# ChainSafe/Spectre

Measured on NVIDIA H100. Metric: bn254_g1_msm_pairs_per_s, higher is better.
Workload: dtype u256 (8x32-bit Montgomery limbs, INT32 IMAD)

## Files before the change

### spectre_b200/csrc/capi.cu

```cuda
#include "common.cuh"
#include "ntt.cuh"
#include "../../include/spectre_b200.h"
#include <stdarg.h>
#include <stdio.h>
#include <sys/types.h>
#include <stdlib.h>
#include <string.h>

using namespace spb;

static_assert(sizeof(spb_fr) == sizeof(Fr) && sizeof(spb_g1_affine) == sizeof(G1Affine) && sizeof(spb_g1) == sizeof(G1Jac),
              "C ABI structs must match the device structs byte for byte");

namespace spb {

int set_error(spb_ctx* ctx, int code, const char* fmt, ...) {
  char buf[512];
  va_list ap; va_start(ap, fmt); vsnprintf(buf, sizeof buf, fmt, ap); va_end(ap);
  if (ctx) ctx->last_error = buf;
  return code;
}

void* slot(spb_ctx* ctx, DeviceState& d, const char* name, size_t bytes) {
  DevBuf& b = d.slots[name];
// ... 78 lines not shown

}

template <class P>
__global__ void field_op_kernel(int op, const Fp<P>* a, const Fp<P>* b, Fp<P>* o, size_t n) {
  size_t i = blockIdx.x * (size_t)blockDim.x + threadIdx.x;
  if (i >= n) return;
  Fp<P> x = a[i], y = b[i], r;
  if (op == 0) r = fp_mul(x, y);
  else if (op == 1) r = fp_add(x, y);
  else r = fp_sub(x, y);
  o[i] = r;
}

template <class P, int ILP, bool SQR = false>
__global__ void modmul_bench_kernel(Fp<P>* out, uint32_t iters) {
  Fp<P> x[ILP], y;
  uint32_t tid = blockIdx.x * blockDim.x + threadIdx.x;
#pragma unroll
  for (int j = 0; j < ILP; j++) { x[j] = fp_one<P>(); x[j].l[0] ^= tid * 2654435761u + j; x[j].l[7] &= 0x0fffffffu; }
  y = x[0]; y.l[1] ^= 0x9e3779b9u;
  for (uint32_t i = 0; i < iters; i++) {
#pragma unroll
    for (int j = 0; j < ILP; j++) x[j] = SQR ? fp_sqr(x[j]) : fp_mul(x[j], y);
  }
  Fp<P> acc = x[0];
#pragma unroll
  for (int j = 1; j < ILP; j++) acc = fp_add(acc, x[j]);
  out[tid] = acc;
}

extern "C" {

int spb_device_count(void) {
  int n = 0;
  if (cudaGetDeviceCount(&n) != cudaSuccess) return 0;
  return n;
}

spb_ctx* spb_init(const int* device_ids, int n_dev) {
  int avail = spb_device_count();
  if (n_dev <= 0) n_dev = 1;
  if (avail <= 0) { fprintf(stderr, "spectre_b200: no CUDA device visible; this library has no CPU fallback\n"); return nullptr; }
  spb_ctx* ctx = new spb_ctx();
  for (int i = 0; i < n_dev; i++) {
    int id = device_ids ? device_ids[i] : i;
    if (id < 0 || id >= avail) { fprintf(stderr, "spectre_b200: device id %d out of range (have %d)\n", id, avail); delete ctx; return nullptr; }
    DeviceState d; d.device = id;
    if (cudaSetDevice(id) != cudaSuccess) { delete ctx; return nullptr; }
    cudaDeviceProp prop;
    if (cudaGetDeviceProperties(&prop, id) != cudaSuccess) { delete ctx; return nullptr; }
    d.sm_count = prop.multiProcessorCount;
    d.total_mem = prop.totalGlobalMem;
    if (cudaStreamCreateWithFlags(&d.stream, cudaStreamNonBlocking) != cudaSuccess) { delete ctx; return nullptr; }
    cudaEventCreate(&d.ev0); cudaEventCreate(&d.ev1);
    cudaEventCreateWithFlags(&d.dep_ev, cudaEventDisableTiming);
    for (int e = 0; e < 8; e++) cudaEventCreate(&d.stage_ev[e]);
    d.pinned_cap = 1 << 20;
    if (cudaMallocHost(&d.pinned, d.pinned_cap) != cudaSuccess) { delete ctx; return nullptr; }
    ctx->dev.push_back(d);
  }
  ctx->peer_access = ctx->dev.size() > 1;
  for (size_t i = 0; i < ctx->dev.size(); i++)
    for (size_t j = 0; j < ctx->dev.size(); j++) {
      if (i == j) continue;
      int can = 0;
      cudaDeviceCanAccessPeer(&can, ctx->dev[i].device, ctx->dev[j].device);
      if (!can) { ctx->peer_access = false; continue; }
      cudaSetDevice(ctx->dev[i].device);
      cudaError_t e = cudaDeviceEnablePeerAccess(ctx->dev[j].device, 0);
      if (e != cudaSuccess && e != cudaErrorPeerAccessAlreadyEnabled) ctx->peer_access = false;
      cudaGetLastError();
    }
  if (!ctx->dev.empty()) cudaSetDevice(ctx->dev[0].device);
  return ctx;
}

void spb_shutdown(spb_ctx* ctx) {
  if (!ctx) return;
  msm_release_ctx(ctx);
  for (auto& d : ctx->dev) {
    cudaSetDevice(d.device);
    cudaStreamSynchronize(d.stream);
    for (auto& kv : d.slots) if (kv.second.ptr) cudaFree(kv.second.ptr);
    ntt_free_tables(d);
    if (d.pinned) cudaFreeHost(d.pinned);
    for (int i = 0; i < 2; i++) { if (d.stage[i]) cudaFreeHost(d.stage[i]); if (d.stage_done[i]) cudaEventDestroy(d.stage_done[i]); }
    cudaEventDestroy(d.ev0); cudaEventDestroy(d.ev1); cudaEventDestroy(d.dep_ev);
    for (int e = 0; e < 8; e++) cudaEventDestroy(d.stage_ev[e]);
    cudaStreamDestroy(d.stream);
  }
  delete ctx;
}

int spb_release_workspace(spb_ctx* ctx) {
  if (!ctx) return SPB_ERR_ARG;
  std::lock_guard<std::mutex> lk(ctx->mu);
  if (ctx->shplonk_slots_busy) return set_error(ctx, SPB_ERR_STATE, "spb_release_workspace: an spb_shplonk handle is open");
  for (auto& d : ctx->dev) {
    SPB_CUDA(ctx, cudaSetDevice(d.device));
    SPB_CUDA(ctx, cudaDeviceSynchronize());
    for (auto& kv : d.slots) if (kv.second.ptr) cudaFree(kv.second.ptr);
    d.slots.clear();
    ntt_free_tables(d);
  }
  if (!ctx->dev.empty()) cudaSetDevice(ctx->dev[0].device);
// ... 301 lines not shown
```

### spectre_b200/csrc/common.cuh

```cuda
#pragma once
#include <cuda_runtime.h>
#include <stdint.h>
#include <stdio.h>
#include <string.h>
#include <initializer_list>
#include <map>
#include <mutex>
#include <string>
#include <vector>
#include "curve.cuh"
#include "../../include/spectre_b200.h"

namespace spb {


struct DevBuf {
  void* ptr = nullptr;
  size_t cap = 0;
};

struct NttTables {
  Fr omega;
  uint32_t k, h;
  Fr* tw_lo = nullptr;
  Fr* tw_hi = nullptr;
  Fr* tw_full = nullptr;
};

struct MsmLane {
  cudaStream_t stream = nullptr;
  cudaEvent_t ev[9] = {nullptr, nullptr, nullptr, nullptr, nullptr, nullptr, nullptr, nullptr, nullptr};
  void* pinned = nullptr;
  bool ready = false;
};
static const int kMaxMsmLanes = 3;

struct DeviceState {
  int device = 0;
  int sm_count = 0;
  size_t total_mem = 0;
  cudaStream_t stream = nullptr;
  cudaEvent_t ev0 = nullptr, ev1 = nullptr;
  cudaEvent_t dep_ev = nullptr;
  cudaEvent_t stage_ev[8] = {nullptr, nullptr, nullptr, nullptr, nullptr, nullptr, nullptr, nullptr};
  std::map<std::string, DevBuf> slots;
  MsmLane lanes[kMaxMsmLanes];
  std::vector<NttTables> ntt_tables;
  std::vector<NttTables> ntt_pre_tables;
  void* pinned = nullptr;
  size_t pinned_cap = 0;
  void* stage[2] = {nullptr, nullptr};
  cudaEvent_t stage_done[2] = {nullptr, nullptr};
};

}

struct spb_ctx {
  std::vector<spb::DeviceState> dev;
  std::mutex mu;
  std::string last_error;
  bool peer_access = false;
  uint64_t n_kernel_launches = 0;
  float last_kernel_ms = 0.f;
  uint64_t last_msm_adds = 0;
  bool shplonk_slots_busy = false;
  float msm_stage_ms[7] = {0, 0, 0, 0, 0, 0, 0};
};

struct spb_domain {
  uint32_t j, k, extended_k, quotient_poly_degree;
  spb::Fr omega, omega_inv, extended_omega, extended_omega_inv, g_coset, g_coset_inv, ifft_divisor, extended_ifft_divisor;
  uint32_t t_len;
  spb::Fr* d_t_evaluations;
  int device;
};

namespace spb {

int set_error(spb_ctx* ctx, int code, const char* fmt, ...);
void* slot(spb_ctx* ctx, DeviceState& d, const char* name, size_t bytes);

#define SPB_CUDA(ctx, call)                                                                      \
  do {                                                                                           \
    cudaError_t e_ = (call);                                                                     \
    if (e_ != cudaSuccess) return spb::set_error(ctx, SPB_ERR_CUDA, "%s:%d %s: %s", __FILE__, __LINE__, #call, cudaGetErrorString(e_)); \
  } while (0)
#define SPB_TRY(expr)            \
  do {                           \
    int rc_ = (expr);            \
    if (rc_ != 0) return rc_;    \
  } while (0)

// ... 2 lines not shown
  DeviceState& d = (ctx)->dev[0];               \
  SPB_CUDA(ctx, cudaSetDevice(d.device));

inline unsigned nblk(uint64_t n, unsigned t) { return (unsigned)((n + t - 1) / t); }

template <class... P, class... A>
int launch(spb_ctx* ctx, cudaStream_t stream, dim3 grid, dim3 block, size_t smem, void (*kernel)(P...), const A&... args) {
  if (!grid.x || !grid.y || !grid.z) return 0;
  kernel<<<grid, block, smem, stream>>>(args...);
  ctx->n_kernel_launches++;
  const cudaError_t e = cudaGetLastError();
  if (e != cudaSuccess)
    return set_error(ctx, SPB_ERR_CUDA, "kernel launch (grid %ux%ux%u, block %u, %zu B shared memory): %s", grid.x, grid.y, grid.z,
                     block.x * block.y * block.z, smem, cudaGetErrorString(e));
  return 0;
}

struct Staging {
  const char* slot;
  size_t bytes;
  const void* in;
  void* out;
  size_t in_bytes = bytes, out_bytes = bytes;
};
template <class Core>
int run_staged(spb_ctx* ctx, DeviceState& d, std::initializer_list<Staging> bufs, Core&& core) {
  std::vector<void*> p;
  for (const Staging& b : bufs) {
    p.push_back(slot(ctx, d, b.slot, b.bytes));
    if (!p.back()) return SPB_ERR_OOM;
  }
  size_t i = 0;
  for (const Staging& b : bufs) {
    if (b.in) SPB_CUDA(ctx, cudaMemcpyAsync(p[i], b.in, b.in_bytes, cudaMemcpyHostToDevice, d.stream));
    i++;
  }
  SPB_TRY(core(p.data()));
  i = 0;
  for (const Staging& b : bufs) {
    if (b.out) SPB_CUDA(ctx, cudaMemcpyAsync(b.out, p[i], b.out_bytes, cudaMemcpyDeviceToHost, d.stream));
    i++;
  }
  SPB_CUDA(ctx, cudaStreamSynchronize(d.stream));
  return 0;
}

struct RowRange { int dev_index; uint64_t lo, hi; };
std::vector<RowRange> row_ranges(spb_ctx* ctx, uint64_t rows);

int stream_file_to_device(spb_ctx* ctx, DeviceState& d, FILE* f, void* d_dst, size_t bytes, const char* what);
int stream_device_to_file(spb_ctx* ctx, DeviceState& d, FILE* f, const void* d_src, size_t bytes, const char* what);

void msm_release_ctx(spb_ctx* ctx);

struct NttOpts {
  uint64_t n_in = 0, n_out = 0;
  const Fr* pre3 = nullptr;
  const Fr* post3 = nullptr;
  const Fr* pre_generator = nullptr;
};
void ntt_free_tables(DeviceState& d);
int ntt_device(spb_ctx* ctx, DeviceState& d, const Fr* d_src, Fr* d_dst, uint32_t log_n, const Fr& omega, const NttOpts& opts);
bool ntt_multi_applicable(spb_ctx* ctx, uint32_t log_n);
int ntt_multi_host(spb_ctx* ctx, const Fr* in, Fr* out, uint32_t log_n, const Fr& omega, const NttOpts& opts, float* ev_ms);

int dev_grand_product(spb_ctx* ctx, DeviceState& d, const Fr* da, size_t n, Fr* dz, const Fr& init);
int dev_kate_division(spb_ctx* ctx, DeviceState& d, const Fr* da, size_t n, const Fr& b, Fr* dq);
int dev_batch_invert(spb_ctx* ctx, DeviceState& d, Fr* da, size_t n);
int dev_product_enqueue(spb_ctx* ctx, DeviceState& d, const Fr* da, size_t n, Fr** d_total);
int dev_eval_polynomial(spb_ctx* ctx, DeviceState& d, const Fr* dp, size_t n, const Fr& x, Fr* out_host);

inline Fr fr_from_u64(uint64_t v) {
  Fr a = fp_zero<FrParams>(); a.l[0] = (uint32_t)v; a.l[1] = (uint32_t)(v >> 32);
  return fp_to_mont(a);
}
inline Fr fr_load(const spb_fr* p) { Fr a; memcpy(&a, p, 32); return a; }
inline Fr fr_const(const uint32_t (&v)[8]) { Fr a; for (int i = 0; i < 8; i++) a.l[i] = v[i]; return a; }
inline Fr fr_root_of_unity(uint32_t k) {
  constexpr uint32_t v[8] = SPB_FR_ROOT_OF_UNITY_MONT;
  Fr w = fr_const(v);
  for (uint32_t i = k; i < SPB_FR_S; i++) w = fp_sqr(w);
  return w;
}
inline Fr fr_zeta() { constexpr uint32_t v[8] = SPB_FR_ZETA_MONT; return fr_const(v); }
inline Fr fr_delta() { constexpr uint32_t v[8] = SPB_FR_DELTA_MONT; return fr_const(v); }

}
```

### spectre_b200/csrc/msm.cu

```cuda
#define SPB_MSM_KERNELS 1
#include "common.cuh"
#include "msm.cuh"
#include <cub/device/device_scan.cuh>
#include <string.h>

using namespace spb;

struct SrsShard {
  int dev_index = 0;
  size_t start = 0, count = 0;
  G1Affine* g = nullptr;
  G1Affine* g_lagrange = nullptr;
};
struct spb_srs {
  uint32_t k = 0;
  size_t n = 0;
  unsigned char g2[128] = {0}, s_g2[128] = {0};
  uint32_t table_c = 0;
  std::vector<SrsShard> shards;
};


namespace spb {

typedef MsmLane Lane;
static const size_t kLanePinnedBytes = 256 * 1024;
static int get_lane(spb_ctx* ctx, int dev_index, int lane_index, Lane** out) {
  Lane& l = ctx->dev[dev_index].lanes[lane_index];
  if (!l.ready) {
    SPB_CUDA(ctx, cudaStreamCreateWithFlags(&l.stream, cudaStreamNonBlocking));
    for (int i = 0; i < 9; i++) SPB_CUDA(ctx, cudaEventCreate(&l.ev[i]));
    SPB_CUDA(ctx, cudaMallocHost(&l.pinned, kLanePinnedBytes));
    l.ready = true;
  }
  *out = &l;
  return 0;
}

void msm_release_ctx(spb_ctx* ctx) {
  for (auto& d : ctx->dev) {
    cudaSetDevice(d.device);
    for (auto& l : d.lanes) {
      if (!l.ready) continue;
      cudaStreamSynchronize(l.stream);
      for (int i = 0; i < 9; i++) cudaEventDestroy(l.ev[i]);
      cudaFreeHost(l.pinned);
      cudaStreamDestroy(l.stream);
      l = Lane();
    }
  }
}

static void* lane_slot(spb_ctx* ctx, DeviceState& d, int lane, const char* name, size_t bytes) {
  char buf[64];
  snprintf(buf, sizeof buf, "%s#%d", name, lane);
  return slot(ctx, d, buf, bytes);
}

static uint32_t choose_chunk(const DeviceState& d, uint64_t est_entries) {
  const double wave = (double)d.sm_count * 512.0;
  if (est_entries >= kLongChunkMinEntries) return kLongChunk;
  double waves = (double)est_entries / 32.0 / wave;
  if (waves < 1.0) return 32;
  double w = waves < 1.5 ? 1.0 : (double)(uint64_t)(waves + 0.5);
  uint32_t L = (uint32_t)((double)est_entries / (w * wave)) + 1;
  if (L < 24) L = 24;
  if (L > 48) L = 48;
  return L;
}

static int msm_enqueue(spb_ctx* ctx, DeviceState& d, int lane, Lane& ln, const Fr* d_scalars, const G1Affine* d_bases, uint64_t n, MsmGeom g) {
  const uint64_t nb = (uint64_t)g.BW * g.B;
  const uint64_t cap = n * g.W;
  const uint32_t Lmin = g.L == kLongChunk ? kShortChunk : g.L;
  const uint64_t Tmax = (cap + Lmin - 1) / Lmin;
  if (cap >= 0x7fffffffull) return set_error(ctx, SPB_ERR_ARG, "msm: %llu entries exceed the 31-bit sort index", (unsigned long long)cap);
  uint32_t* counts = (uint32_t*)lane_slot(ctx, d, lane, "msm_counts", (nb + 1) * 4);
  uint32_t* offsets = (uint32_t*)lane_slot(ctx, d, lane, "msm_offsets", (nb + 1) * 4);
  MsmEntry* ent = (MsmEntry*)lane_slot(ctx, d, lane, "msm_entries", (cap + 1) * sizeof(MsmEntry));
  G1Xyzz* buckets = (G1Xyzz*)lane_slot(ctx, d, lane, "msm_buckets", nb * sizeof(G1Xyzz));
  uint32_t* head_key = (uint32_t*)lane_slot(ctx, d, lane, "msm_head_key", (Tmax + 1) * 4);
  uint32_t* tail_key = (uint32_t*)lane_slot(ctx, d, lane, "msm_tail_key", (Tmax + 1) * 4);
  G1Xyzz* head = (G1Xyzz*)lane_slot(ctx, d, lane, "msm_head", (Tmax + 1) * sizeof(G1Xyzz));
  G1Xyzz* tail = (G1Xyzz*)lane_slot(ctx, d, lane, "msm_tail", (Tmax + 1) * sizeof(G1Xyzz));
  uint32_t* giant = (uint32_t*)lane_slot(ctx, d, lane, "msm_giant", (Tmax + 2) * 4);
  const uint64_t max_huge = Tmax / kHugeChain + 1;
  uint32_t* huge = (uint32_t*)lane_slot(ctx, d, lane, "msm_huge", (2 * max_huge + 2) * 4);
  G1Xyzz* huge_part = (G1Xyzz*)lane_slot(ctx, d, lane, "msm_huge_part", max_huge * kHugeBlocks * sizeof(G1Xyzz));
  const MsmTail tl = msm_tail_shape(g.c);
  const uint32_t R = 1u << tl.r_log, C = 1u << tl.c_log, per = msm_tail_partials(tl);
  const uint32_t T1 = g.B >> tl.m_log;
  const uint64_t ngroups = (uint64_t)g.BW * T1;
  G1Xyzz* grp = (G1Xyzz*)lane_slot(ctx, d, lane, "msm_groups", 2 * ngroups * sizeof(G1Xyzz));
  G1Xyzz* seg_out = (G1Xyzz*)lane_slot(ctx, d, lane, "msm_rowcol", (uint64_t)g.BW * (2 * R + C) * sizeof(G1Xyzz));
  G1Xyzz* win_out = (G1Xyzz*)lane_slot(ctx, d, lane, "msm_partials", (uint64_t)g.BW * per * sizeof(G1Xyzz));
  size_t scan_bytes = 0;
  cub::DeviceScan::ExclusiveSum(nullptr, scan_bytes, counts, offsets, (int)(nb + 1), ln.stream);
  void* scan_tmp = lane_slot(ctx, d, lane, "msm_scan_tmp", scan_bytes ? scan_bytes : 16);
  if (!counts || !offsets || !ent || !buckets || !head_key || !tail_key || !head || !tail || !giant || !huge || !huge_part || !grp || !seg_out || !win_out || !scan_tmp)
    return SPB_ERR_OOM;
  if ((size_t)g.BW * per * sizeof(G1Xyzz) + 16 > kLanePinnedBytes) return set_error(ctx, SPB_ERR_STATE, "msm: %u window partials exceed the pinned staging area", g.BW * per);

  cudaStream_t st = ln.stream;
  SPB_CUDA(ctx, cudaMemsetAsync(giant, 0, 4, st));
  SPB_CUDA(ctx, cudaMemsetAsync(huge, 0, 4, st));
  const unsigned tb = 256;
  SPB_CUDA(ctx, cudaMemsetAsync(counts, 0, (nb + 1) * 4, st));
  cudaEventRecord(ln.ev[0], st);
  SPB_TRY(launch(ctx, st, nblk(n, tb), tb, 0, msm_count_kernel, n, d_scalars, g, counts));
  cudaEventRecord(ln.ev[1], st);
  SPB_CUDA(ctx, cub::DeviceScan::ExclusiveSum(scan_tmp, scan_bytes, counts, offsets, (int)(nb + 1), st));
  SPB_CUDA(ctx, cudaMemcpyAsync(counts, offsets, (nb + 1) * 4, cudaMemcpyDeviceToDevice, st));
  cudaEventRecord(ln.ev[2], st);
  SPB_TRY(launch(ctx, st, nblk(n, tb), tb, 0, msm_scatter_kernel, n, d_scalars, g, counts, ent));
  const uint32_t* total = offsets + nb;
  cudaEventRecord(ln.ev[3], st);
  SPB_TRY(launch(ctx, st, nblk(Tmax, 128), 128, 0, msm_accumulate_kernel, total, g, ent, d_bases, buckets, head_key, head, tail_key, tail));
  cudaEventRecord(ln.ev[4], st);
  SPB_TRY(launch(ctx, st, nblk(Tmax, 128), 128, 0, msm_stitch_kernel, total, g.L, 24, head_key, head, tail_key, tail, buckets, giant, giant + 1));
  SPB_TRY(launch(ctx, st, 256, 128, 0, msm_giant_kernel, total, g.L, giant, giant + 1, head_key, head, tail_key, tail, buckets, huge, huge + 2));
  SPB_TRY(launch(ctx, st, kHugeBlocks, 128, 0, msm_huge_kernel, huge, huge + 2, head, huge_part));
  SPB_TRY(launch(ctx, st, 64, 128, 0, msm_huge_finish_kernel, huge, huge + 2, kHugeBlocks, huge_part, tail_key, tail, buckets));
  cudaEventRecord(ln.ev[5], st);
  G1Xyzz *rows = seg_out, *cols = seg_out + (uint64_t)g.BW * R, *wrows = seg_out + (uint64_t)g.BW * (R + C);
  SPB_TRY(launch(ctx, st, nblk(ngroups, 128), 128, 0, msm_group_kernel, ngroups, tl.m_log, offsets, buckets, grp, grp + ngroups));
  cudaEventRecord(ln.ev[6], st);
  SPB_TRY(launch(ctx, st, g.BW * (2 * R + C), 64, 0, msm_rowcol_kernel, T1, tl, grp, grp + ngroups, rows, cols, wrows));
  SPB_TRY(launch(ctx, st, g.BW * (2 * tl.nbr + tl.nbc), 128, 0, msm_weighted_kernel, tl, rows, cols, wrows, win_out));
  cudaEventRecord(ln.ev[7], st);
  SPB_CUDA(ctx, cudaMemcpyAsync(ln.pinned, win_out, (size_t)g.BW * per * sizeof(G1Xyzz), cudaMemcpyDeviceToHost, st));
  SPB_CUDA(ctx, cudaMemcpyAsync((char*)ln.pinned + (size_t)g.BW * per * sizeof(G1Xyzz), total, 4, cudaMemcpyDeviceToHost, st));
  return 0;
}

static G1Xyzz msm_finish(Lane& ln, MsmGeom g, uint64_t* adds) {
  const MsmTail tl = msm_tail_shape(g.c);
  const uint32_t per = msm_tail_partials(tl);
  const G1Xyzz* P = (const G1Xyzz*)ln.pinned;
  uint32_t M; memcpy(&M, (const char*)ln.pinned + (size_t)g.BW * per * sizeof(G1Xyzz), 4);
  if (adds) *adds += (uint64_t)M + 2ull * g.BW * g.B;
  std::vector<G1Xyzz> S(g.BW);
  for (uint32_t w = 0; w < g.BW; w++) S[w] = msm_tail_finish(g, P + (size_t)w * per);
  return msm_combine_windows(S.data(), g.BW, g.c);
}

static void write_result(const G1Xyzz& r, spb_g1* out) {
  G1Affine a = xyzz_to_affine(r);
  G1Jac j = jac_from_affine(a);
  memcpy(out, &j, sizeof(G1Jac));
}

struct MsmPart {
  int dev_index;
  const Fr* d_scalars;
  const Fr* h_scalars;
  int peer_src_device;
  const G1Affine* d_bases;
  uint64_t n;
  MsmGeom g;
};

static int job_enqueue(spb_ctx* ctx, int lane, std::vector<MsmPart>& parts) {
  for (auto& p : parts) {
    if (!p.n) continue;
    DeviceState& d = ctx->dev[p.dev_index];
    SPB_CUDA(ctx, cudaSetDevice(d.device));
    Lane* ln; SPB_TRY(get_lane(ctx, p.dev_index, lane, &ln));
    p.g.L = choose_chunk(d, p.n * p.g.W);
    const Fr* ds = p.d_scalars;
    DeviceState& src = p.peer_src_device >= 0 ? ctx->dev[0] : d;
    if (&src != &d) SPB_CUDA(ctx, cudaSetDevice(src.device));
    SPB_CUDA(ctx, cudaEventRecord(src.dep_ev, src.stream));
    if (&src != &d) SPB_CUDA(ctx, cudaSetDevice(d.device));
// ... 363 lines not shown
    if (!src) return set_error(ctx, SPB_ERR_STATE, "spb_srs_download: basis %d not resident", basis);
    DeviceState& d = ctx->dev[sh.dev_index];
    SPB_CUDA(ctx, cudaSetDevice(d.device));
    SPB_CUDA(ctx, cudaMemcpy((G1Affine*)out + (lo - start), src + (lo - sh.start), (hi - lo) * sizeof(G1Affine), cudaMemcpyDeviceToHost));
  }
  return 0;
}

int spb_msm_raw(spb_ctx* ctx, const spb_fr* scalars, const spb_g1_affine* bases, size_t n, spb_g1* out) {
  if (!ctx || !out || (n && (!scalars || !bases))) return SPB_ERR_ARG;
  std::lock_guard<std::mutex> lk(ctx->mu);
  ctx->last_msm_adds = 0;
  std::vector<MsmPart> parts;
  size_t D = ctx->dev.size();
  for (size_t i = 0; i < D; i++) {
    size_t lo = n * i / D, cnt = n * (i + 1) / D - lo;
    if (!cnt) continue;
    DeviceState& d = ctx->dev[i];
    SPB_CUDA(ctx, cudaSetDevice(d.device));
    Lane* ln; SPB_TRY(get_lane(ctx, (int)i, 0, &ln));
    G1Affine* db = (G1Affine*)slot(ctx, d, "msm_raw_bases", cnt * sizeof(G1Affine));
    if (!db) return SPB_ERR_OOM;
    SPB_CUDA(ctx, cudaMemcpyAsync(db, (const G1Affine*)bases + lo, cnt * sizeof(G1Affine), cudaMemcpyHostToDevice, ln->stream));
    MsmPart p; p.dev_index = (int)i; p.d_scalars = nullptr; p.h_scalars = (const Fr*)scalars + lo; p.peer_src_device = -1;
    p.d_bases = db; p.n = cnt; p.g = msm_choose_geometry(cnt);
    parts.push_back(p);
  }
  SPB_TRY(job_enqueue(ctx, 0, parts));
  return job_collect(ctx, 0, parts, out);
}

static int srs_parts(spb_ctx* ctx, const spb_srs* srs, int basis, const Fr* scalars, bool on_device, size_t n, std::vector<MsmPart>& parts) {
  if (n > srs->n) return set_error(ctx, SPB_ERR_ARG, "spb_msm: %zu scalars but the SRS has %zu points", n, srs->n);
  for (auto& sh : srs->shards) {
    if (sh.start >= n) continue;
    size_t cnt = (n - sh.start) < sh.count ? (n - sh.start) : sh.count;
    const G1Affine* b = basis == SPB_BASIS_G ? sh.g : sh.g_lagrange;
    if (!b) return set_error(ctx, SPB_ERR_STATE, "spb_msm: basis %d not resident", basis);
    MsmPart p; p.dev_index = sh.dev_index; p.d_bases = b; p.n = cnt; p.h_scalars = nullptr; p.d_scalars = nullptr; p.peer_src_device = -1;
    if (!on_device) p.h_scalars = scalars + sh.start;
    else { p.d_scalars = scalars + sh.start; if (sh.dev_index != 0) p.peer_src_device = ctx->dev[0].device; }
    p.g = srs->table_c ? msm_make_geometry(srs->table_c, true, (uint32_t)sh.count) : msm_choose_geometry(cnt);
    parts.push_back(p);
  }
  return 0;
}

static int msm_batch_common(spb_ctx* ctx, const spb_srs* srs, int basis, const spb_fr* const* scalars, bool on_device, size_t n, size_t count, spb_g1* out) {
  if (!ctx || !srs || !out || (count && !scalars)) return SPB_ERR_ARG;
  std::lock_guard<std::mutex> lk(ctx->mu);
  ctx->last_msm_adds = 0;
  const MsmGeom lg = srs->table_c ? msm_make_geometry(srs->table_c, true, 0) : msm_choose_geometry(n ? n : 1);
  const uint64_t ents = (uint64_t)n * lg.W;
  const uint64_t lane_bytes = ents * sizeof(MsmEntry) + 2 * (ents / kShortChunk + 1) * (sizeof(G1Xyzz) + 4) + (uint64_t)lg.BW * lg.B * sizeof(G1Xyzz);
  const uint64_t fit = ctx->dev[0].total_mem / 10 / (lane_bytes ? lane_bytes : 1);
  const size_t NL = std::max<size_t>(1, std::min<size_t>((size_t)kMaxMsmLanes, (size_t)fit));
  std::vector<MsmPart> jobs[kMaxMsmLanes];
  for (size_t i = 0; i < count; i++) {
    int lane = (int)(i % NL);
    if (i >= NL) SPB_TRY(job_collect(ctx, lane, jobs[lane], &out[i - NL]));
    if (n && !scalars[i]) return SPB_ERR_ARG;
    jobs[lane].clear();
    SPB_TRY(srs_parts(ctx, srs, basis, (const Fr*)scalars[i], on_device, n, jobs[lane]));
    SPB_TRY(job_enqueue(ctx, lane, jobs[lane]));
  }
  for (size_t i = count >= NL ? count - NL : 0; i < count; i++) SPB_TRY(job_collect(ctx, (int)(i % NL), jobs[i % NL], &out[i]));
  return 0;
}

int spb_msm(spb_ctx* ctx, const spb_srs* srs, int basis, const spb_fr* scalars, size_t n, spb_g1* out) {
  const spb_fr* one[1] = {scalars};
  if (n && !scalars) return SPB_ERR_ARG;
  return msm_batch_common(ctx, srs, basis, one, false, n, 1, out);
}
int spb_msm_dev(spb_ctx* ctx, const spb_srs* srs, int basis, const spb_fr* d_scalars, size_t n, spb_g1* out) {
  const spb_fr* one[1] = {d_scalars};
  if (n && !d_scalars) return SPB_ERR_ARG;
  return msm_batch_common(ctx, srs, basis, one, true, n, 1, out);
}
int spb_msm_batch(spb_ctx* ctx, const spb_srs* srs, int basis, const spb_fr* const* scalars, size_t n, size_t count, spb_g1* out) {
  return msm_batch_common(ctx, srs, basis, scalars, false, n, count, out);
}
int spb_msm_batch_dev(spb_ctx* ctx, const spb_srs* srs, int basis, const spb_fr* const* d_scalars, size_t n, size_t count, spb_g1* out) {
  return msm_batch_common(ctx, srs, basis, d_scalars, true, n, count, out);
}

int spb_srs_precompute(spb_ctx* ctx, spb_srs* srs) {
  if (!ctx || !srs) return SPB_ERR_ARG;
  std::lock_guard<std::mutex> lk(ctx->mu);
  if (srs->table_c) return 0;
  size_t per_dev = srs->shards.empty() ? srs->n : srs->shards[0].count;
  uint32_t c = msm_choose_c(per_dev ? per_dev : 1, true);
  uint32_t W = (255 + c - 1) / c;
  for (auto& sh : srs->shards) {
    if (!sh.count) continue;
    SPB_CUDA(ctx, cudaSetDevice(ctx->dev[sh.dev_index].device));
    size_t free_b = 0, total_b = 0;
    SPB_CUDA(ctx, cudaMemGetInfo(&free_b, &total_b));
    const size_t bases = (sh.g ? 1 : 0) + (sh.g_lagrange ? 1 : 0);
    if ((size_t)W * sh.count * sizeof(G1Affine) * bases > total_b / 4) return 0;
  }
  for (auto& sh : srs->shards) {
    if (!sh.count) continue;
    DeviceState& d = ctx->dev[sh.dev_index];
    SPB_CUDA(ctx, cudaSetDevice(d.device));
    if ((uint64_t)W * sh.count >= 0x7fffffffull) return set_error(ctx, SPB_ERR_ARG, "spb_srs_precompute: table index exceeds 31 bits");
    for (int which = 0; which < 2; which++) {
// ... 26 lines not shown
```

### spectre_b200/csrc/msm.cuh

```cuda
#pragma once
#include <stdlib.h>
#include "curve.cuh"

namespace spb {

struct MsmGeom {
  uint32_t c;
  uint32_t W;
  uint32_t B;
  uint32_t L;
  uint32_t BW;
  uint32_t precomp;
  uint32_t tab_stride;
};

struct alignas(8) MsmEntry { uint32_t key, val; };

static const uint32_t kLongChunk = 96, kShortChunk = 32;
#ifndef SPB_LONG_CHUNK_MIN_ENTRIES
#define SPB_LONG_CHUNK_MIN_ENTRIES (1ull << 23)
#endif
static const uint64_t kLongChunkMinEntries = SPB_LONG_CHUNK_MIN_ENTRIES;
SPB_HD uint32_t msm_effective_chunk(uint32_t L, uint64_t M) { return (L == kLongChunk && M < kLongChunkMinEntries) ? kShortChunk : L; }

static const uint32_t kNoKey = 0xffffffffu;

#if defined(__CUDA_ARCH__)
SPB_D uint32_t spb_atomic_inc(uint32_t* p) { return atomicAdd(p, 1u); }
#else
inline uint32_t spb_atomic_inc(uint32_t* p) { uint32_t v = *p; *p = v + 1; return v; }
#endif

struct DigitIter {
  uint32_t limbs[8];
  uint32_t c, carry, w;
  SPB_HD void init(const Fr& canonical, uint32_t c_) {
    for (int i = 0; i < 8; i++) limbs[i] = canonical.l[i];
    c = c_; carry = 0; w = 0;
  }
  SPB_HD int32_t next() {
    uint32_t bit = w * c, word = bit >> 5, sh = bit & 31;
    uint64_t v = 0;
    if (word < 8) {
      v = limbs[word];
      if (word + 1 < 8) v |= (uint64_t)limbs[word + 1] << 32;
      v >>= sh;
    }
    uint32_t raw = (uint32_t)(v & ((1u << c) - 1)) + carry;
    w++;
    if (raw > (1u << (c - 1))) { carry = 1; return (int32_t)raw - (int32_t)(1u << c); }
    carry = 0;
    return (int32_t)raw;
  }
};

SPB_HD void msm_count_thread(uint64_t tid, uint64_t n, const Fr* scalars, MsmGeom g, uint32_t* counts) {
  if (tid >= n) return;
  Fr s = fp_from_mont(scalars[tid]);
  if (fp_is_zero(s)) return;
  DigitIter it; it.init(s, g.c);
  for (uint32_t w = 0; w < g.W; w++) {
    int32_t d = it.next();
    if (d == 0) continue;
    uint32_t mag = d < 0 ? (uint32_t)(-d) : (uint32_t)d;
    spb_atomic_inc(&counts[(g.precomp ? 0u : w * g.B) + mag - 1]);
  }
}

SPB_HD void msm_scatter_thread(uint64_t tid, uint64_t n, const Fr* scalars, MsmGeom g, uint32_t* cursor, MsmEntry* ent) {
  if (tid >= n) return;
  Fr s = fp_from_mont(scalars[tid]);
  if (fp_is_zero(s)) return;
  DigitIter it; it.init(s, g.c);
  for (uint32_t w = 0; w < g.W; w++) {
    int32_t d = it.next();
    if (d == 0) continue;
    uint32_t mag = d < 0 ? (uint32_t)(-d) : (uint32_t)d;
    uint32_t key = (g.precomp ? 0u : w * g.B) + mag - 1;
    uint32_t pos = spb_atomic_inc(&cursor[key]);
    MsmEntry e; e.key = key; e.val = ((uint32_t)tid + (g.precomp ? w * g.tab_stride : 0u)) | (d < 0 ? 0x80000000u : 0u);
    ent[pos] = e;
  }
}

SPB_HD G1Affine msm_load_point(const G1Affine* bases, uint32_t val) {
#if defined(__CUDA_ARCH__)
  const uint4* q = reinterpret_cast<const uint4*>(bases + (val & 0x7fffffffu));
  uint4 a = __ldg(q), b = __ldg(q + 1), c = __ldg(q + 2), d = __ldg(q + 3);
  G1Affine p;
  p.x.l[0] = a.x; p.x.l[1] = a.y; p.x.l[2] = a.z; p.x.l[3] = a.w; p.x.l[4] = b.x; p.x.l[5] = b.y; p.x.l[6] = b.z; p.x.l[7] = b.w;
  p.y.l[0] = c.x; p.y.l[1] = c.y; p.y.l[2] = c.z; p.y.l[3] = c.w; p.y.l[4] = d.x; p.y.l[5] = d.y; p.y.l[6] = d.z; p.y.l[7] = d.w;
#else
  G1Affine p = bases[val & 0x7fffffffu];
#endif
  if (val & 0x80000000u) p.y = fp_neg(p.y);
  return p;
}

SPB_HD MsmEntry msm_load_entry(const MsmEntry* p) {
#if defined(__CUDA_ARCH__)
  uint2 v = __ldg(reinterpret_cast<const uint2*>(p));
  MsmEntry e; e.key = v.x; e.val = v.y; return e;
#else
  return *p;
#endif
}

SPB_HD void msm_accumulate_thread(uint64_t tid, uint64_t M, MsmGeom g, const MsmEntry* ent,
                                  const G1Affine* bases, G1Xyzz* buckets, uint32_t* head_key, G1Xyzz* head,
                                  uint32_t* tail_key, G1Xyzz* tail) {
  const uint32_t L = msm_effective_chunk(g.L, M);
  uint64_t lo = tid * L;
  if (lo >= M) return;
  uint64_t hi = lo + L < M ? lo + L : M;
  uint32_t hk = kNoKey, tk = kNoKey;
  MsmEntry first = msm_load_entry(ent + lo);
  uint32_t cur = first.key;
  bool run_started_before = lo > 0 && msm_load_entry(ent + lo - 1).key == cur;
  G1Xyzz acc = xyzz_from_affine(msm_load_point(bases, first.val));
  for (uint64_t e = lo + 1; e < hi; e++) {
    MsmEntry en = msm_load_entry(ent + e);
    uint32_t k = en.key;
    G1Affine p = msm_load_point(bases, en.val);
    if (k == cur) {
      xyzz_add_mixed(acc, p);
    } else {
      if (run_started_before) { hk = cur; head[tid] = acc; }
      else buckets[cur] = acc;
      run_started_before = false;
      cur = k;
      acc = xyzz_from_affine(p);
    }
  }
  bool continues = hi < M && msm_load_entry(ent + hi).key == cur;
  if (continues) {
    if (run_started_before) { hk = cur; head[tid] = acc; }
    else { tk = cur; tail[tid] = acc; }
  } else {
    if (run_started_before) { hk = cur; head[tid] = acc; }
    else buckets[cur] = acc;
  }
  head_key[tid] = hk;
  tail_key[tid] = tk;
}

SPB_HD void msm_stitch_thread(uint64_t tid, uint64_t T, uint32_t cap, const uint32_t* head_key, const G1Xyzz* head,
                              const uint32_t* tail_key, const G1Xyzz* tail, G1Xyzz* buckets, uint32_t* giant_count,
                              uint32_t* giant_list) {
  if (tid >= T) return;
  uint32_t key = tail_key[tid];
  if (key == kNoKey) return;
  uint64_t j = tid + 1, len = 0;
  while (j < T && head_key[j] == key && len <= cap) { j++; len++; }
  if (len > cap) { uint32_t slot = spb_atomic_inc(giant_count); giant_list[slot] = (uint32_t)tid; return; }
  G1Xyzz acc = tail[tid];
  for (uint64_t q = tid + 1; q < tid + 1 + len; q++) xyzz_add(acc, head[q]);
  buckets[key] = acc;
}

struct MsmTail {
  uint32_t m_log;
  uint32_t r_log, c_log;
  uint32_t nbr, nbc;
};
inline MsmTail msm_tail_shape(uint32_t c) {
  MsmTail t; uint32_t bits = c - 1;
  t.m_log = bits < 3 ? bits : 3;
  bits -= t.m_log;
  t.c_log = bits / 2; t.r_log = bits - t.c_log;
  t.nbr = ((1u << t.r_log) + 127) / 128; t.nbc = ((1u << t.c_log) + 127) / 128;
  return t;
}
SPB_HD uint32_t msm_tail_partials(const MsmTail& t) { return 3 * t.nbr + 2 * t.nbc; }

SPB_HD void msm_group_thread(uint64_t tid, uint64_t ngroups, uint32_t m_log, const uint32_t* offsets, const G1Xyzz* buckets, G1Xyzz* s1, G1Xyzz* w1) {
  if (tid >= ngroups) return;
  const uint64_t b0 = tid << m_log;
  G1Xyzz run = xyzz_identity(), acc = xyzz_identity();
  uint32_t hi = offsets[b0 + (1u << m_log)];
  for (int j = (int)(1u << m_log) - 1; j >= 0; j--) {
    const uint32_t lo = offsets[b0 + (uint64_t)j];
    if (hi != lo) xyzz_add(run, buckets[b0 + (uint64_t)j]);
    hi = lo;
    if (j >= 1) xyzz_add(acc, run);
  }
  s1[tid] = run;
  w1[tid] = acc;
}
inline void msm_tail_host(const MsmGeom& g, const uint32_t* offsets, const G1Xyzz* buckets, G1Xyzz* partials) {
  MsmTail t = msm_tail_shape(g.c);
  uint32_t R = 1u << t.r_log, C = 1u << t.c_log, per = msm_tail_partials(t);
  const uint64_t T = (uint64_t)g.B >> t.m_log;
  G1Xyzz* s1 = (G1Xyzz*)malloc(sizeof(G1Xyzz) * T * g.BW);
  G1Xyzz* w1 = (G1Xyzz*)malloc(sizeof(G1Xyzz) * T * g.BW);
  for (uint64_t tid = 0; tid < T * g.BW; tid++) msm_group_thread(tid, T * g.BW, t.m_log, offsets, buckets, s1, w1);
  for (uint32_t w = 0; w < g.BW; w++) {
// ... 43 lines not shown
  return A;
}

#if defined(__CUDACC__) && defined(SPB_MSM_KERNELS)
__device__ __forceinline__ unsigned msm_warp_peers(uint32_t key, uint32_t lane) {
  const uint32_t next = __shfl_down_sync(0xffffffffu, key, 1);
  const bool dup = lane < 31u && next == key && key != kNoKey;
  if (__any_sync(0xffffffffu, dup)) return __match_any_sync(0xffffffffu, key);
  return 1u << lane;
}
__global__ void msm_count_kernel(uint64_t n, const Fr* scalars, MsmGeom g, uint32_t* counts) {
  const uint64_t tid = blockIdx.x * (uint64_t)blockDim.x + threadIdx.x;
  const uint32_t lane = threadIdx.x & 31u;
  bool live = tid < n;
  Fr s = live ? fp_from_mont(scalars[tid]) : fp_zero<FrParams>();
  live = live && !fp_is_zero(s);
  DigitIter it; it.init(s, g.c);
  for (uint32_t w = 0; w < g.W; w++) {
    int32_t d = it.next();
    const bool act = live && d != 0;
    const uint32_t mag = d < 0 ? (uint32_t)(-d) : (uint32_t)d;
    const uint32_t key = (g.precomp ? 0u : w * g.B) + mag - 1;
    const unsigned peers = msm_warp_peers(act ? key : kNoKey, lane);
    if (act && lane == (uint32_t)(__ffs(peers) - 1)) atomicAdd(&counts[key], (uint32_t)__popc(peers));
  }
}
__global__ void msm_scatter_kernel(uint64_t n, const Fr* scalars, MsmGeom g, uint32_t* cursor, MsmEntry* ent) {
  const uint64_t tid = blockIdx.x * (uint64_t)blockDim.x + threadIdx.x;
  const uint32_t lane = threadIdx.x & 31u;
  bool live = tid < n;
  Fr s = live ? fp_from_mont(scalars[tid]) : fp_zero<FrParams>();
  live = live && !fp_is_zero(s);
  DigitIter it; it.init(s, g.c);
  for (uint32_t w = 0; w < g.W; w++) {
    int32_t d = it.next();
    const bool act = live && d != 0;
    const uint32_t mag = d < 0 ? (uint32_t)(-d) : (uint32_t)d;
    const uint32_t key = (g.precomp ? 0u : w * g.B) + mag - 1;
    const unsigned peers = msm_warp_peers(act ? key : kNoKey, lane);
    const uint32_t leader = (uint32_t)(__ffs(peers) - 1);
    uint32_t base = 0;
    if (act && lane == leader) base = atomicAdd(&cursor[key], (uint32_t)__popc(peers));
    base = __shfl_sync(0xffffffffu, base, leader);
    if (act) {
      const uint32_t pos = base + (uint32_t)__popc(peers & ((1u << lane) - 1u));
      MsmEntry e; e.key = key; e.val = ((uint32_t)tid + (g.precomp ? w * g.tab_stride : 0u)) | (d < 0 ? 0x80000000u : 0u);
      ent[pos] = e;
    }
  }
}
#ifndef SPB_ACC_MINBLOCKS
#define SPB_ACC_MINBLOCKS 1
#endif
__global__ void __launch_bounds__(128, SPB_ACC_MINBLOCKS) msm_accumulate_kernel(const uint32_t* total, MsmGeom g, const MsmEntry* ent,
                                                             const G1Affine* bases, G1Xyzz* buckets, uint32_t* head_key, G1Xyzz* head,
                                                             uint32_t* tail_key, G1Xyzz* tail) {
  msm_accumulate_thread(blockIdx.x * (uint64_t)blockDim.x + threadIdx.x, *total, g, ent, bases, buckets, head_key, head, tail_key, tail);
}
__global__ void __launch_bounds__(128) msm_stitch_kernel(const uint32_t* total, uint32_t L, uint32_t cap, const uint32_t* head_key, const G1Xyzz* head,
                                                         const uint32_t* tail_key, const G1Xyzz* tail, G1Xyzz* buckets, uint32_t* giant_count, uint32_t* giant_list) {
  L = msm_effective_chunk(L, *total);
  uint64_t T = ((uint64_t)*total + L - 1) / L;
  msm_stitch_thread(blockIdx.x * (uint64_t)blockDim.x + threadIdx.x, T, cap, head_key, head, tail_key, tail, buckets, giant_count, giant_list);
}

template <int NT>
__device__ void block_sum_xyzz(G1Xyzz& v, G1Xyzz* sh) {
  const int tid = threadIdx.x;
  for (int stride = NT / 2; stride >= 1; stride >>= 1) {
    if (tid >= stride && tid < 2 * stride) sh[tid - stride] = v;
    __syncthreads();
    if (tid < stride) xyzz_add(v, sh[tid]);
    __syncthreads();
  }
}

template <int NT>
__device__ void block_sum2_xyzz(G1Xyzz& a, G1Xyzz& b, G1Xyzz* sh ) {
  const int tid = threadIdx.x;
  for (int stride = NT / 2; stride >= 1; stride >>= 1) {
    if (tid >= stride && tid < 2 * stride) { sh[2 * (tid - stride)] = a; sh[2 * (tid - stride) + 1] = b; }
    __syncthreads();
    if (tid < stride) { xyzz_add(a, sh[2 * tid]); xyzz_add(b, sh[2 * tid + 1]); }
    __syncthreads();
  }
}

static const uint32_t kHugeChain = 4096;
static const uint32_t kHugeBlocks = 1056;
__global__ void __launch_bounds__(128) msm_giant_kernel(const uint32_t* total, uint32_t L, const uint32_t* giant_count, const uint32_t* giant_list,
                                                        const uint32_t* head_key, const G1Xyzz* head, const uint32_t* tail_key, const G1Xyzz* tail,
                                                        G1Xyzz* buckets, uint32_t* huge_count, uint32_t* huge_list ) {
  __shared__ G1Xyzz sh[64];
  __shared__ uint64_t s_end;
  L = msm_effective_chunk(L, *total);
  const uint64_t T = ((uint64_t)*total + L - 1) / L;
  const uint32_t count = *giant_count;
  for (uint32_t gi = blockIdx.x; gi < count; gi += gridDim.x) {
    uint64_t t0 = giant_list[gi];
    uint32_t key = tail_key[t0];
    if (threadIdx.x == 0) {
      uint64_t lo = t0 + 1, hi = T;
      while (lo < hi) { uint64_t mid = (lo + hi) >> 1; if (head_key[mid] == key) lo = mid + 1; else hi = mid; }
      s_end = lo;
    }
    __syncthreads();
    const uint64_t end = s_end;
    if (end - (t0 + 1) > kHugeChain) {
      if (threadIdx.x == 0) { uint32_t slot = atomicAdd(huge_count, 1u); huge_list[2 * slot] = (uint32_t)t0; huge_list[2 * slot + 1] = (uint32_t)end; }
      __syncthreads();
      continue;
    }
    G1Xyzz acc = xyzz_identity();
    for (uint64_t j = t0 + 1 + threadIdx.x; j < end; j += 128) xyzz_add(acc, head[j]);
    block_sum_xyzz<128>(acc, sh);
    if (threadIdx.x == 0) { xyzz_add(acc, tail[t0]); buckets[key] = acc; }
    __syncthreads();
  }
}
__global__ void __launch_bounds__(128) msm_huge_kernel(const uint32_t* huge_count, const uint32_t* huge_list, const G1Xyzz* head, G1Xyzz* partial) {
  __shared__ G1Xyzz sh[64];
  const uint32_t count = *huge_count;
  if (!count) return;
  const uint32_t nparts = gridDim.x / count ? gridDim.x / count : 1;
  for (uint64_t work = blockIdx.x; work < (uint64_t)count * nparts; work += gridDim.x) {
    const uint32_t hi = (uint32_t)(work / nparts), part = (uint32_t)(work % nparts);
    const uint64_t t0 = huge_list[2 * hi], end = huge_list[2 * hi + 1];
    G1Xyzz acc = xyzz_identity();
    for (uint64_t j = t0 + 1 + (uint64_t)part * 128 + threadIdx.x; j < end; j += (uint64_t)nparts * 128) xyzz_add(acc, head[j]);
    block_sum_xyzz<128>(acc, sh);
    if (threadIdx.x == 0) partial[(uint64_t)hi * gridDim.x + part] = acc;
    __syncthreads();
  }
}
__global__ void __launch_bounds__(128) msm_huge_finish_kernel(const uint32_t* huge_count, const uint32_t* huge_list, uint32_t grid_parts, const G1Xyzz* partial,
                                                              const uint32_t* tail_key, const G1Xyzz* tail, G1Xyzz* buckets) {
  __shared__ G1Xyzz sh[64];
  const uint32_t count = *huge_count;
  if (!count) return;
  const uint32_t nparts = grid_parts / count ? grid_parts / count : 1;
  for (uint32_t hi = blockIdx.x; hi < count; hi += gridDim.x) {
    G1Xyzz acc = xyzz_identity();
    for (uint32_t j = threadIdx.x; j < nparts; j += 128) xyzz_add(acc, partial[(uint64_t)hi * grid_parts + j]);
    block_sum_xyzz<128>(acc, sh);
    const uint64_t t0 = huge_list[2 * hi];
    if (threadIdx.x == 0) { xyzz_add(acc, tail[t0]); buckets[tail_key[t0]] = acc; }
    __syncthreads();
  }
}
// ... 160 lines not shown
```

Measured before the change: 294.5 million.

## Shrink MSM accumulate chunk length so small inputs fill all resident threads

Queries occupancy of the accumulate kernel at init and stores the number of resident threads per device. The accumulate, stitch and giant kernels now compute the chunk length as the minimum of the configured chunk and ceil(M/resident_threads), so small MSMs are split over enough threads to fill the GPU. Chunk-count bounds and lane memory estimates are raised to match. In exchange there are more chunk heads and tails to stitch, and more partial-sum traffic.

```diff
diff --git a/spectre_b200/csrc/capi.cu b/spectre_b200/csrc/capi.cu
--- a/spectre_b200/csrc/capi.cu
+++ b/spectre_b200/csrc/capi.cu
@@ -154,6 +154,7 @@
     if (cudaGetDeviceProperties(&prop, id) != cudaSuccess) { delete ctx; return nullptr; }
     d.sm_count = prop.multiProcessorCount;
     d.total_mem = prop.totalGlobalMem;
+    if (msm_query_resident(d) != cudaSuccess) { delete ctx; return nullptr; }
     if (cudaStreamCreateWithFlags(&d.stream, cudaStreamNonBlocking) != cudaSuccess) { delete ctx; return nullptr; }
     cudaEventCreate(&d.ev0); cudaEventCreate(&d.ev1);
     cudaEventCreateWithFlags(&d.dep_ev, cudaEventDisableTiming);
diff --git a/spectre_b200/csrc/common.cuh b/spectre_b200/csrc/common.cuh
--- a/spectre_b200/csrc/common.cuh
+++ b/spectre_b200/csrc/common.cuh
@@ -38,6 +38,7 @@
 struct DeviceState {
   int device = 0;
   int sm_count = 0;
+  uint64_t msm_acc_threads = 0;
   size_t total_mem = 0;
   cudaStream_t stream = nullptr;
   cudaEvent_t ev0 = nullptr, ev1 = nullptr;
@@ -146,6 +147,7 @@
 int stream_device_to_file(spb_ctx* ctx, DeviceState& d, FILE* f, const void* d_src, size_t bytes, const char* what);
 
 void msm_release_ctx(spb_ctx* ctx);
+cudaError_t msm_query_resident(DeviceState& d);
 
 struct NttOpts {
   uint64_t n_in = 0, n_out = 0;
diff --git a/spectre_b200/csrc/msm.cu b/spectre_b200/csrc/msm.cu
--- a/spectre_b200/csrc/msm.cu
+++ b/spectre_b200/csrc/msm.cu
@@ -57,6 +57,19 @@
   return slot(ctx, d, buf, bytes);
 }
 
+cudaError_t msm_query_resident(DeviceState& d) {
+  int per_sm = 0;
+  const cudaError_t e = cudaOccupancyMaxActiveBlocksPerMultiprocessor(&per_sm, msm_accumulate_kernel, 128, 0);
+  if (e != cudaSuccess) return e;
+  d.msm_acc_threads = (uint64_t)d.sm_count * (uint64_t)(per_sm > 1 ? per_sm : 1) * 128;
+  return cudaSuccess;
+}
+
+static uint64_t msm_max_chunks(const DeviceState& d, uint64_t entries, uint32_t Lmin) {
+  const uint64_t fixed = (entries + Lmin - 1) / Lmin, fill = entries < d.msm_acc_threads ? entries : d.msm_acc_threads;
+  return fixed > fill ? fixed : fill;
+}
+
 static uint32_t choose_chunk(const DeviceState& d, uint64_t est_entries) {
   const double wave = (double)d.sm_count * 512.0;
   if (est_entries >= kLongChunkMinEntries) return kLongChunk;
@@ -73,7 +86,7 @@
   const uint64_t nb = (uint64_t)g.BW * g.B;
   const uint64_t cap = n * g.W;
   const uint32_t Lmin = g.L == kLongChunk ? kShortChunk : g.L;
-  const uint64_t Tmax = (cap + Lmin - 1) / Lmin;
+  const uint64_t Tmax = msm_max_chunks(d, cap, Lmin);
   if (cap >= 0x7fffffffull) return set_error(ctx, SPB_ERR_ARG, "msm: %llu entries exceed the 31-bit sort index", (unsigned long long)cap);
   uint32_t* counts = (uint32_t*)lane_slot(ctx, d, lane, "msm_counts", (nb + 1) * 4);
   uint32_t* offsets = (uint32_t*)lane_slot(ctx, d, lane, "msm_offsets", (nb + 1) * 4);
@@ -115,10 +128,10 @@
   SPB_TRY(launch(ctx, st, nblk(n, tb), tb, 0, msm_scatter_kernel, n, d_scalars, g, counts, ent));
   const uint32_t* total = offsets + nb;
   cudaEventRecord(ln.ev[3], st);
-  SPB_TRY(launch(ctx, st, nblk(Tmax, 128), 128, 0, msm_accumulate_kernel, total, g, ent, d_bases, buckets, head_key, head, tail_key, tail));
+  SPB_TRY(launch(ctx, st, nblk(Tmax, 128), 128, 0, msm_accumulate_kernel, total, g, d.msm_acc_threads, ent, d_bases, buckets, head_key, head, tail_key, tail));
   cudaEventRecord(ln.ev[4], st);
-  SPB_TRY(launch(ctx, st, nblk(Tmax, 128), 128, 0, msm_stitch_kernel, total, g.L, 24, head_key, head, tail_key, tail, buckets, giant, giant + 1));
-  SPB_TRY(launch(ctx, st, 256, 128, 0, msm_giant_kernel, total, g.L, giant, giant + 1, head_key, head, tail_key, tail, buckets, huge, huge + 2));
+  SPB_TRY(launch(ctx, st, nblk(Tmax, 128), 128, 0, msm_stitch_kernel, total, g.L, d.msm_acc_threads, 24, head_key, head, tail_key, tail, buckets, giant, giant + 1));
+  SPB_TRY(launch(ctx, st, 256, 128, 0, msm_giant_kernel, total, g.L, d.msm_acc_threads, giant, giant + 1, head_key, head, tail_key, tail, buckets, huge, huge + 2));
   SPB_TRY(launch(ctx, st, kHugeBlocks, 128, 0, msm_huge_kernel, huge, huge + 2, head, huge_part));
   SPB_TRY(launch(ctx, st, 64, 128, 0, msm_huge_finish_kernel, huge, huge + 2, kHugeBlocks, huge_part, tail_key, tail, buckets));
   cudaEventRecord(ln.ev[5], st);
@@ -588,7 +601,7 @@
   ctx->last_msm_adds = 0;
   const MsmGeom lg = srs->table_c ? msm_make_geometry(srs->table_c, true, 0) : msm_choose_geometry(n ? n : 1);
   const uint64_t ents = (uint64_t)n * lg.W;
-  const uint64_t lane_bytes = ents * sizeof(MsmEntry) + 2 * (ents / kShortChunk + 1) * (sizeof(G1Xyzz) + 4) + (uint64_t)lg.BW * lg.B * sizeof(G1Xyzz);
+  const uint64_t lane_bytes = ents * sizeof(MsmEntry) + 2 * (msm_max_chunks(ctx->dev[0], ents, kShortChunk) + 1) * (sizeof(G1Xyzz) + 4) + (uint64_t)lg.BW * lg.B * sizeof(G1Xyzz);
   const uint64_t fit = ctx->dev[0].total_mem / 10 / (lane_bytes ? lane_bytes : 1);
   const size_t NL = std::max<size_t>(1, std::min<size_t>((size_t)kMaxMsmLanes, (size_t)fit));
   std::vector<MsmPart> jobs[kMaxMsmLanes];
diff --git a/spectre_b200/csrc/msm.cuh b/spectre_b200/csrc/msm.cuh
--- a/spectre_b200/csrc/msm.cuh
+++ b/spectre_b200/csrc/msm.cuh
@@ -22,6 +22,11 @@
 #endif
 static const uint64_t kLongChunkMinEntries = SPB_LONG_CHUNK_MIN_ENTRIES;
 SPB_HD uint32_t msm_effective_chunk(uint32_t L, uint64_t M) { return (L == kLongChunk && M < kLongChunkMinEntries) ? kShortChunk : L; }
+SPB_HD uint64_t msm_kernel_chunk(uint32_t L, uint64_t M, uint64_t fill_threads) {
+  const uint64_t Le = msm_effective_chunk(L, M), Lf = M > fill_threads ? (M + fill_threads - 1) / fill_threads : 1;
+  return Lf < Le ? Lf : Le;
+}
+SPB_HD uint64_t msm_kernel_chunks(uint32_t L, uint64_t M, uint64_t fill_threads) { const uint64_t c = msm_kernel_chunk(L, M, fill_threads); return (M + c - 1) / c; }
 
 static const uint32_t kNoKey = 0xffffffffu;
 
@@ -106,10 +111,9 @@
 #endif
 }
 
-SPB_HD void msm_accumulate_thread(uint64_t tid, uint64_t M, MsmGeom g, const MsmEntry* ent,
-                                  const G1Affine* bases, G1Xyzz* buckets, uint32_t* head_key, G1Xyzz* head,
-                                  uint32_t* tail_key, G1Xyzz* tail) {
-  const uint32_t L = msm_effective_chunk(g.L, M);
+SPB_HD void msm_accumulate_chunk(uint64_t tid, uint64_t L, uint64_t M, const MsmEntry* ent,
+                                 const G1Affine* bases, G1Xyzz* buckets, uint32_t* head_key, G1Xyzz* head,
+                                 uint32_t* tail_key, G1Xyzz* tail) {
   uint64_t lo = tid * L;
   if (lo >= M) return;
   uint64_t hi = lo + L < M ? lo + L : M;
@@ -142,6 +146,15 @@
   }
   head_key[tid] = hk;
   tail_key[tid] = tk;
+}
+SPB_HD void msm_accumulate_fill_thread(uint64_t tid, uint64_t M, MsmGeom g, uint64_t fill_threads, const MsmEntry* ent, const G1Affine* bases,
+                                       G1Xyzz* buckets, uint32_t* head_key, G1Xyzz* head, uint32_t* tail_key, G1Xyzz* tail) {
+  msm_accumulate_chunk(tid, msm_kernel_chunk(g.L, M, fill_threads), M, ent, bases, buckets, head_key, head, tail_key, tail);
+}
+SPB_HD void msm_accumulate_thread(uint64_t tid, uint64_t M, MsmGeom g, const MsmEntry* ent,
+                                  const G1Affine* bases, G1Xyzz* buckets, uint32_t* head_key, G1Xyzz* head,
+                                  uint32_t* tail_key, G1Xyzz* tail) {
+  msm_accumulate_chunk(tid, msm_effective_chunk(g.L, M), M, ent, bases, buckets, head_key, head, tail_key, tail);
 }
 
 SPB_HD void msm_stitch_thread(uint64_t tid, uint64_t T, uint32_t cap, const uint32_t* head_key, const G1Xyzz* head,
@@ -291,15 +304,14 @@
 #ifndef SPB_ACC_MINBLOCKS
 #define SPB_ACC_MINBLOCKS 1
 #endif
-__global__ void __launch_bounds__(128, SPB_ACC_MINBLOCKS) msm_accumulate_kernel(const uint32_t* total, MsmGeom g, const MsmEntry* ent,
+__global__ void __launch_bounds__(128, SPB_ACC_MINBLOCKS) msm_accumulate_kernel(const uint32_t* total, MsmGeom g, uint64_t fill_threads, const MsmEntry* ent,
                                                              const G1Affine* bases, G1Xyzz* buckets, uint32_t* head_key, G1Xyzz* head,
                                                              uint32_t* tail_key, G1Xyzz* tail) {
-  msm_accumulate_thread(blockIdx.x * (uint64_t)blockDim.x + threadIdx.x, *total, g, ent, bases, buckets, head_key, head, tail_key, tail);
-}
-__global__ void __launch_bounds__(128) msm_stitch_kernel(const uint32_t* total, uint32_t L, uint32_t cap, const uint32_t* head_key, const G1Xyzz* head,
+  msm_accumulate_fill_thread(blockIdx.x * (uint64_t)blockDim.x + threadIdx.x, *total, g, fill_threads, ent, bases, buckets, head_key, head, tail_key, tail);
+}
+__global__ void __launch_bounds__(128) msm_stitch_kernel(const uint32_t* total, uint32_t L, uint64_t fill_threads, uint32_t cap, const uint32_t* head_key, const G1Xyzz* head,
                                                          const uint32_t* tail_key, const G1Xyzz* tail, G1Xyzz* buckets, uint32_t* giant_count, uint32_t* giant_list) {
-  L = msm_effective_chunk(L, *total);
-  uint64_t T = ((uint64_t)*total + L - 1) / L;
+  const uint64_t T = msm_kernel_chunks(L, *total, fill_threads);
   msm_stitch_thread(blockIdx.x * (uint64_t)blockDim.x + threadIdx.x, T, cap, head_key, head, tail_key, tail, buckets, giant_count, giant_list);
 }
 
@@ -327,13 +339,12 @@
 
 static const uint32_t kHugeChain = 4096;
 static const uint32_t kHugeBlocks = 1056;
-__global__ void __launch_bounds__(128) msm_giant_kernel(const uint32_t* total, uint32_t L, const uint32_t* giant_count, const uint32_t* giant_list,
+__global__ void __launch_bounds__(128) msm_giant_kernel(const uint32_t* total, uint32_t L, uint64_t fill_threads, const uint32_t* giant_count, const uint32_t* giant_list,
                                                         const uint32_t* head_key, const G1Xyzz* head, const uint32_t* tail_key, const G1Xyzz* tail,
                                                         G1Xyzz* buckets, uint32_t* huge_count, uint32_t* huge_list ) {
   __shared__ G1Xyzz sh[64];
   __shared__ uint64_t s_end;
-  L = msm_effective_chunk(L, *total);
-  const uint64_t T = ((uint64_t)*total + L - 1) / L;
+  const uint64_t T = msm_kernel_chunks(L, *total, fill_threads);
   const uint32_t count = *giant_count;
   for (uint32_t gi = blockIdx.x; gi < count; gi += gridDim.x) {
     uint64_t t0 = giant_list[gi];
```

Result: no change. 293.2 million (median of 6 runs) (-0.4%).
